# YihongSun/Dynamo-Depth

Measured on AMD Instinct MI355X. Metric: training images/sec (192x640 triplets), higher is better.
Workload: dtype f32

## Files before the change

dynamo-depth_amd/csrc/dd_pw_gemm.hip:

```cpp
#include <hip/hip_runtime.h>
#include <type_traits>

#include "../../include/dynamo_hip.h"
#include "dd_attr.h"
#include "dd_split.h"
#include "dd_store_tile.h"

namespace dd {
namespace pw {

using cm::bf8;
using cm::f16v;
using cm::split2;
using cm::store_acc32;
using cm::StoreF32;
using cm::tile_bias;

constexpr int FRAG_U4 = 64;

struct PackRegion {
  const float* w;
  long long s_n, s_k;
  int N, K, first;
  int fused;
// ... 324 lines not shown
    for (int n = 0; n < NB2; ++n)
      store_acc32<decltype(full)::value>(acc2[n], bv[n], y + (size_t)row * C + n * 32 + (lane & 31), (size_t)C, M - row, StoreF32{});
  };
  if ((int)blockIdx.x * 128 + 128 <= M) tail(std::true_type{});
  else tail(std::false_type{});
}

template <int C>
static int launch_fused(const float* x, const void* pack1, const void* pack2, const float* b1, const float* b2, int M, float* y, hipStream_t stream) {
  constexpr int lds = ((C / 16) * 3 + (C / 32) * 6) * FRAG + 6 * C * 4;
  auto kern = mlp_fwd_kernel<C>;
  static dd::LdsAttrOnce lds_attr;
  if (const int rc = lds_attr.ensure(reinterpret_cast<const void*>(kern), (int)(lds))) return rc;
  hipLaunchKernelGGL(kern, dim3((M + 127) / 128), dim3(256), lds, stream, x, static_cast<const uint4*>(pack1), static_cast<const uint4*>(pack2), b1, b2, M, y);
  return (int)hipGetLastError();
}

constexpr int C3 = 224, KS3 = C3 / 16, NB3 = C3 / 32, NHB3 = 6 * C3 / 32;
constexpr int NF3 = KS3 * 3;
constexpr int BR3 = (NF3 + 3) / 4;
constexpr int MLP3_LDS = 2 * NF3 * FRAG + 6 * C3 * 4;
static_assert(NF3 == NB3 * 6, "both operands of a hidden block have the same number of fragments");

template <int NP>
__global__ __launch_bounds__(256, 1) void mlp_fwd224_kernel(const float* __restrict__ x, const uint4* __restrict__ pack1, const uint4* __restrict__ pack2,
                                                            const float* __restrict__ b1, const float* __restrict__ bias, int M, int S,
                                                            float* __restrict__ dst) {
  extern __shared__ __align__(16) unsigned char smem[];
  unsigned char* const s_w1 = smem;
  unsigned char* const s_w2 = smem + NF3 * FRAG;
  float* const s_b1 = reinterpret_cast<float*>(smem + 2 * NF3 * FRAG);
  const int tid = threadIdx.x, lane = tid & 63, wave = __builtin_amdgcn_readfirstlane(tid >> 6) & 3, hh = lane >> 5;
  const int row0 = (int)blockIdx.x * 128 + wave * 32;
  const int split = (int)blockIdx.y, hb0 = split * NHB3 / S, hb1 = (split + 1) * NHB3 / S;

  for (int i = tid; i < 6 * C3; i += 256) s_b1[i] = b1[i];
  uint4 xf[KS3][3];
  {
    const float* xp = x + (size_t)min(row0 + (lane & 31), M - 1) * C3 + hh * 8;
#pragma unroll
    for (int ks = 0; ks < KS3; ++ks) {
      const float4 v0 = *reinterpret_cast<const float4*>(xp + ks * 16), v1 = *reinterpret_cast<const float4*>(xp + ks * 16 + 4);
      unsigned p[3][4];
      split2(v0.x, v0.y, p[0][0], p[1][0], p[2][0]);
      split2(v0.z, v0.w, p[0][1], p[1][1], p[2][1]);
      split2(v1.x, v1.y, p[0][2], p[1][2], p[2][2]);
      split2(v1.z, v1.w, p[0][3], p[1][3], p[2][3]);
#pragma unroll
      for (int pc = 0; pc < 3; ++pc) xf[ks][pc] = make_uint4(p[pc][0], p[pc][1], p[pc][2], p[pc][3]);
    }
  }
  const unsigned lds0 = (unsigned)reinterpret_cast<size_t>(smem);
  auto dma = [&](const uint4* pack, int hb, unsigned char* s_w) {
    const uint4* src = pack + (size_t)hb * (NF3 * 64) + lane;
#pragma unroll
    for (int r = 0; r < BR3; ++r) {
      const int f = min(wave + 4 * r, NF3 - 1);
      const unsigned dst = __builtin_amdgcn_readfirstlane(lds0 + (unsigned)(s_w - smem) + f * FRAG);
      unsigned keep;
      asm volatile("s_mov_b32 %0, m0\n\ts_mov_b32 m0, %2\n\ts_nop 0\n\tglobal_load_lds_dwordx4 %1, off\n\ts_mov_b32 m0, %0"
                   : "=&s"(keep) : "v"(src + f * 64), "s"(dst) : "memory");
    }
  };
  auto wait_barrier = [&]() { asm volatile("s_waitcnt vmcnt(0) lgkmcnt(0)\n\ts_barrier" ::: "memory"); };

  f16v acc2[NB3];
#pragma unroll
  for (int n = 0; n < NB3; ++n)
#pragma unroll
    for (int r = 0; r < 16; ++r) acc2[n][r] = 0.f;
  auto read_w = [&](const unsigned char* s_w, int f, uint4 (&wf)[3]) {
#pragma unroll
    for (int pc = 0; pc < 3; ++pc) wf[pc] = *reinterpret_cast<const uint4*>(s_w + lane * 16 + (f * 3 + pc) * FRAG);
  };
  float hv[16];
  uint4 hf[2][3];
  auto slice = [&](const f16v& acc, int hb, int i) {
    const int r = i < 11 ? i : i - 3;
    if (i < 11 || (i >= 14 && i < 19)) {
      hv[r] = gelu_erf(acc[r] + s_b1[hb * 32 + 8 * (r >> 2) + 4 * hh + (r & 3)]);
      asm volatile("" : "+v"(hv[r]));
    }
    if (i == 11 || i == 12 || i == 19 || i == 20) {
      const int j = i >= 19, q0 = (i == 12 || i == 20) ? 2 : 0;
      unsigned p[3][2];
#pragma unroll
      for (int q = 0; q < 2; ++q) {
        split2(hv[8 * j + 2 * (q0 + q)], hv[8 * j + 2 * (q0 + q) + 1], p[0][q], p[1][q], p[2][q]);
        asm volatile("" : "+v"(p[0][q]), "+v"(p[1][q]), "+v"(p[2][q]));
      }
#pragma unroll
      for (int pc = 0; pc < 3; ++pc) {
        if (q0 == 0) { hf[j][pc].x = p[pc][0]; hf[j][pc].y = p[pc][1]; }
        else { hf[j][pc].z = p[pc][0]; hf[j][pc].w = p[pc][1]; }
      }
    }
  };
  auto gemm1 = [&](f16v& acc, const f16v& prev, int hb, auto act) {
#pragma unroll
    for (int r = 0; r < 16; ++r) acc[r] = 0.f;
    uint4 wf[2][3];
    read_w(s_w1, 0, wf[0]);
#pragma unroll
    for (int ks = 0; ks < KS3; ++ks) {
      if (ks + 1 < KS3) read_w(s_w1, ks + 1, wf[(ks + 1) & 1]);
#pragma unroll
      for (int t = 6 - NP; t < 6; ++t)
        acc = __builtin_amdgcn_mfma_f32_32x32x16_bf16(__builtin_bit_cast(bf8, wf[ks & 1][cm::kPieceA[t]]), __builtin_bit_cast(bf8, xf[ks][cm::kPieceB[t]]), acc, 0, 0, 0);
      if (decltype(act)::value) slice(prev, hb, ks);
      __builtin_amdgcn_sched_barrier(0);
    }
  };
  auto gemm2 = [&](const f16v& prev, int hb) {
    uint4 wf[2][3];
    read_w(s_w2, 0, wf[0]);
#pragma unroll
    for (int i = 0; i < 2 * NB3; ++i) {
      const int j = i / NB3, n = i - j * NB3;
      if (i + 1 < 2 * NB3) read_w(s_w2, ((i + 1) % NB3) * 2 + (i + 1) / NB3, wf[(i + 1) & 1]);
#pragma unroll
      for (int t = 6 - NP; t < 6; ++t)
        acc2[n] = __builtin_amdgcn_mfma_f32_32x32x16_bf16(__builtin_bit_cast(bf8, hf[j][cm::kPieceA[t]]), __builtin_bit_cast(bf8, wf[i & 1][cm::kPieceB[t]]), acc2[n], 0, 0, 0);
      if (j == 0) slice(prev, hb, 14 + n);
      __builtin_amdgcn_sched_barrier(0);
    }
  };

  float bv[NB3];
#pragma unroll
  for (int n = 0; n < NB3; ++n) bv[n] = tile_bias(bias, n * 32 + (lane & 31), C3, pack2);

  f16v acc1;
  dma(pack1, hb0, s_w1);
  wait_barrier();
  gemm1(acc1, acc1, hb0, std::false_type{});
  wait_barrier();
  dma(pack1, min(hb0 + 1, hb1 - 1), s_w1);
  wait_barrier();
  dma(pack2, hb0, s_w2);
  auto block = [&](int hb, auto more) {
    f16v accn;
    if (decltype(more)::value) gemm1(accn, acc1, hb, std::true_type{});
    else {
#pragma unroll
      for (int i = 0; i < KS3; ++i) slice(acc1, hb, i);
    }
    wait_barrier();
    if (decltype(more)::value) dma(pack1, min(hb + 2, hb1 - 1), s_w1);
    gemm2(acc1, hb);
    if (decltype(more)::value) {
      wait_barrier();
      dma(pack2, hb + 1, s_w2);
#pragma unroll
      for (int r = 0; r < 16; ++r) acc1[r] = accn[r];
    }
  };
  for (int hb = hb0; hb < hb1 - 1; ++hb) block(hb, std::true_type{});
  block(hb1 - 1, std::false_type{});

  float* const out = dst + (size_t)split * M * C3;
  auto tail = [&](auto full) {
    const int row = row0 + 4 * hh;
#pragma unroll
    for (int n = 0; n < NB3; ++n)
      store_acc32<decltype(full)::value>(acc2[n], bv[n], out + (size_t)row * C3 + n * 32 + (lane & 31), (size_t)C3, M - row, StoreF32{});
  };
  if ((int)blockIdx.x * 128 + 128 <= M) tail(std::true_type{});
  else tail(std::false_type{});
}

__global__ __launch_bounds__(256) void mlp_fold224_kernel(const float4* __restrict__ partial, const float4* __restrict__ b2, int S, size_t quads, float4* __restrict__ y) {
  const size_t i = (size_t)blockIdx.x * 256 + threadIdx.x;
  if (i >= quads) return;
  float4 a = b2[i % (C3 / 4)];
  for (int s = 0; s < S; ++s) {
    const float4 p = partial[(size_t)s * quads + i];
    a.x += p.x; a.y += p.y; a.z += p.z; a.w += p.w;
  }
  y[i] = a;
}

static int mlp224_splits(int M) {
  const int groups = (M + 127) / 128, n = 256 / groups;
  return n < 1 ? 1 : n > NHB3 ? NHB3 : n;
}

template <int NP>
static int launch_fused224(const float* x, const void* pack1, const void* pack2, const float* b1, const float* b2, int M, int S, float* y, float* partial,
                           hipStream_t stream) {
  auto kern = mlp_fwd224_kernel<NP>;
  static dd::LdsAttrOnce lds_attr;
  if (const int rc = lds_attr.ensure(reinterpret_cast<const void*>(kern), MLP3_LDS)) return rc;
  hipLaunchKernelGGL(kern, dim3((M + 127) / 128, S), dim3(256), MLP3_LDS, stream, x, static_cast<const uint4*>(pack1), static_cast<const uint4*>(pack2), b1,
                     S == 1 ? b2 : nullptr, M, S, S == 1 ? y : partial);
  if (S == 1) return (int)hipGetLastError();
  const size_t quads = (size_t)M * (C3 / 4);
  hipLaunchKernelGGL(mlp_fold224_kernel, dim3((unsigned)((quads + 255) / 256)), dim3(256), 0, stream, reinterpret_cast<const float4*>(partial),
                     reinterpret_cast<const float4*>(b2), S, quads, reinterpret_cast<float4*>(y));
  return (int)hipGetLastError();
}

__global__ __launch_bounds__(256) void gelu_pair_kernel(const float4* __restrict__ pre, float4* __restrict__ g, float4* __restrict__ post, size_t quads) {
  const size_t i = (size_t)blockIdx.x * 256 + threadIdx.x;
  if (i >= quads) return;
  const float4 x4 = pre[i], g4 = g[i];
  const float xv[4] = {x4.x, x4.y, x4.z, x4.w}, gv[4] = {g4.x, g4.y, g4.z, g4.w};
  float pv[4], dv[4];
#pragma unroll
  for (int e = 0; e < 4; ++e) {
    const float x = xv[e];
    const float er = 1.f + erf_poly(x * 0.70710678118654752440f);
    const float pdf = __expf(-0.5f * x * x) * 0.3989422804014327f;
    pv[e] = (x * 0.5f) * er;
    dv[e] = gv[e] * fmaf(x, pdf, 0.5f * er);
  }
  post[i] = make_float4(pv[0], pv[1], pv[2], pv[3]);
  g[i] = make_float4(dv[0], dv[1], dv[2], dv[3]);
// ... 10 lines not shown
  if (!w1 || !w2 || C < 1 || hidden < 1) return (int)hipErrorInvalidValue;
  PackArgs a;
  a.count = 0;
  a.total = 0;
  bool bad = false;
  auto add = [&](const float* w, long long s_n, long long s_k, int N, int K, void* out, int fused = 0) {
    if (!out) return;
    if (K < 16 || K % 16 || (fused && K % 32)) { bad = true; return; }
    PackRegion& r = a.r[a.count++];
    r.w = w; r.s_n = s_n; r.s_k = s_k; r.N = N; r.K = K; r.first = a.total; r.fused = fused; r.out = static_cast<uint4*>(out);
    a.total += ((N + 31) / 32) * (K / 16);
  };
  add(w1, s1_n, s1_k, hidden, C, pack_fwd1);
  add(w2, s2_n, s2_k, C, hidden, pack_fwd2);
  add(w2, s2_k, s2_n, hidden, C, pack_bwd2);
  add(w1, s1_k, s1_n, C, hidden, pack_bwd1);
  add(w2, s2_n, s2_k, C, hidden, pack_fwd2_fused, 1);
  if (a.count == 0 || bad) return (int)hipErrorInvalidValue;
  for (int i = a.count; i < MAX_REGIONS; ++i) a.r[i] = a.r[0];
  hipLaunchKernelGGL(pw_pack_kernel, dim3((a.total * 64 + 255) / 256), dim3(256), 0, static_cast<hipStream_t>(stream), a);
  return (int)hipGetLastError();
}

extern "C" int dd_mlp_fwd_supported(int C) { return (C == 64 || C == 128 || C == 224) ? 1 : 0; }

extern "C" int dd_mlp_fwd_splits(int M, int C) { return (C == dd::pw::C3 && M >= 1) ? dd::pw::mlp224_splits(M) : 1; }

extern "C" size_t dd_mlp_fwd_workspace_bytes(int M, int C, int splits) {
  if (M < 1 || !dd_mlp_fwd_supported(C) || splits < 0 || splits > dd::pw::NHB3) return 0;
  const int S = splits ? splits : dd_mlp_fwd_splits(M, C);
  return (C == dd::pw::C3 && S > 1) ? (size_t)S * M * C * sizeof(float) : 0;
}

extern "C" int dd_mlp_fwd_n(const float* x, const void* pack_fwd1, const void* pack_fwd2_fused, const float* b1, const float* b2, int M, int C, int products,
                            int splits, float* y, void* workspace, size_t workspace_bytes, void* stream) {
  using namespace dd::pw;
  if (C != C3) return (products == 6 && splits <= 1) ? dd_mlp_fwd(x, pack_fwd1, pack_fwd2_fused, b1, b2, M, C, y, stream) : (int)hipErrorInvalidValue;
  if (!x || !pack_fwd1 || !pack_fwd2_fused || !b1 || !b2 || !y || M < 1 || splits < 0 || splits > NHB3) return (int)hipErrorInvalidValue;
  if (products != 6 && products != 3 && products != 1) return (int)hipErrorInvalidValue;
  if ((reinterpret_cast<unsigned long long>(x) | reinterpret_cast<unsigned long long>(y) | reinterpret_cast<unsigned long long>(b2) |
       reinterpret_cast<unsigned long long>(workspace)) & 15ull)
    return (int)hipErrorInvalidValue;
  const int S = splits ? splits : mlp224_splits(M);
  if (S > 1 && (!workspace || workspace_bytes < dd_mlp_fwd_workspace_bytes(M, C, S))) return (int)hipErrorInvalidValue;
  hipStream_t s = static_cast<hipStream_t>(stream);
  float* part = static_cast<float*>(workspace);
  return products == 6 ? launch_fused224<6>(x, pack_fwd1, pack_fwd2_fused, b1, b2, M, S, y, part, s)
       : products == 3 ? launch_fused224<3>(x, pack_fwd1, pack_fwd2_fused, b1, b2, M, S, y, part, s)
                       : launch_fused224<1>(x, pack_fwd1, pack_fwd2_fused, b1, b2, M, S, y, part, s);
}

extern "C" int dd_mlp_fwd(const float* x, const void* pack_fwd1, const void* pack_fwd2_fused, const float* b1, const float* b2, int M, int C, float* y, void* stream) {
  if (!x || !pack_fwd1 || !pack_fwd2_fused || !b1 || !b2 || !y || M < 1 || (reinterpret_cast<unsigned long long>(x) & 15ull)) return (int)hipErrorInvalidValue;
  hipStream_t s = static_cast<hipStream_t>(stream);
  switch (C) {
    case 64: return dd::pw::launch_fused<64>(x, pack_fwd1, pack_fwd2_fused, b1, b2, M, y, s);
    case 128: return dd::pw::launch_fused<128>(x, pack_fwd1, pack_fwd2_fused, b1, b2, M, y, s);
    case 224: return dd::pw::launch_fused224<6>(x, pack_fwd1, pack_fwd2_fused, b1, b2, M, 1, y, nullptr, s);
    default: return (int)hipErrorInvalidValue;
  }
}

extern "C" int dd_gelu_pair(const float* pre, float* g_inout, float* post, size_t n, void* stream) {
  if (!pre || !g_inout || !post || n == 0 || (n & 3)) return (int)hipErrorInvalidValue;
  if ((reinterpret_cast<unsigned long long>(pre) | reinterpret_cast<unsigned long long>(g_inout) | reinterpret_cast<unsigned long long>(post)) & 15ull)
    return (int)hipErrorInvalidValue;
  const size_t quads = n >> 2;
  hipLaunchKernelGGL(dd::pw::gelu_pair_kernel, dim3((unsigned)((quads + 255) / 256)), dim3(256), 0, static_cast<hipStream_t>(stream),
                     reinterpret_cast<const float4*>(pre), reinterpret_cast<float4*>(g_inout), reinterpret_cast<float4*>(post), quads);
  return (int)hipGetLastError();
}

extern "C" int dd_pw_gemm(const float* x, const void* pack, const float* bias, int M, int K, int N, int gelu_in, float* y, void* stream) {
  using namespace dd::pw;
  if (!x || !pack || !y || M < 1 || K < 32 || K % 32 || N < 1) return (int)hipErrorInvalidValue;
  if ((reinterpret_cast<unsigned long long>(x) & 15ull) || (size_t)M * K >= (1ull << 40) || (size_t)M * N >= (1ull << 40)) return (int)hipErrorInvalidValue;
  hipStream_t s = static_cast<hipStream_t>(stream);
  return gelu_in ? dd::pw::dispatch<true>(x, pack, bias, M, K, N, y, s) : dd::pw::dispatch<false>(x, pack, bias, M, K, N, y, s);
}
```

dynamo-depth_amd/hipops/abi.py:

```python
import ctypes as C

DD_MAX_SCALES = 4
DD_NUM_SRC = 2
DD_ABI_VERSION = 2
DD_MODE_RIGID, DD_MODE_FLOW, DD_MODE_FLOW_MASK = 0, 1, 2
DD_PARTIAL_STRIDE = 40
DD_SUMS_STRIDE = 8

_fp = C.c_void_p


class DDPhotoScale(C.Structure):
    _fields_ = [
        ("shift", C.c_int), ("h", C.c_int), ("w", C.c_int),
        ("w_photo", C.c_float), ("w_cons", C.c_float),
        ("disp", _fp),
        ("flow", _fp * DD_NUM_SRC),
        ("mask", _fp * DD_NUM_SRC),
        ("noise", _fp),
        ("g_disp", _fp),
        ("g_flow", _fp * DD_NUM_SRC),
        ("g_mask", _fp * DD_NUM_SRC),
        ("out_color", _fp * DD_NUM_SRC),
        ("out_sample", _fp * DD_NUM_SRC),
# ... 192 lines not shown
        "dd_conv3x3_mfma_n": (i, [v, v, v, i, i, i, i, i, i, i, v, v]),
        "dd_conv3x3_mfma_flat_supported": (i, [i, i, i, i, i]),
        "dd_conv3x3_mfma_flat_workspace_bytes": (z, [i, i, i, i, i]),
        "dd_conv3x3_mfma_flat": (i, [v, v, v, i, i, i, i, i, v, v, z, v]),
        "dd_conv3x3_mfma_flat_n": (i, [v, v, v, i, i, i, i, i, i, v, v, z, v]),
        "dd_conv3x3_mfma_wgrad_workspace_bytes": (z, [i, i, i, i, i]),
        "dd_conv3x3_mfma_bwd_weight": (i, [v, v, i, i, i, i, i, i, v, v, z, v]),
        "dd_conv3x3_mfma_bwd_weight_n": (i, [v, v, i, i, i, i, i, i, i, v, v, z, v]),
        "dd_conv3x3_half_supported": (i, [i, i]),
        "dd_conv3x3_half_pack_bytes": (z, [i, i]),
        "dd_conv3x3_half_pack": (i, [v, C.c_longlong, C.c_longlong, C.c_longlong, C.c_longlong, i, i, i, v, v, v]),
        "dd_conv3x3_half": (i, [v, v, v, i, i, i, i, i, i, i, v, v]),
        "dd_conv3x3_half_wgrad_workspace_bytes": (z, [i, i, i, i, i]),
        "dd_conv3x3_half_bwd_weight": (i, [v, v, i, i, i, i, i, i, i, v, v, z, v]),
        "dd_pw_gemm_pack_bytes": (z, [i, i]),
        "dd_mlp_pack": (i, [v, C.c_longlong, C.c_longlong, v, C.c_longlong, C.c_longlong, i, i, v, v, v, v, v, v]),
        "dd_mlp_fwd_supported": (i, [i]),
        "dd_mlp_fwd": (i, [v, v, v, v, v, i, i, v, v]),
        "dd_mlp_fwd_splits": (i, [i, i]),
        "dd_mlp_fwd_workspace_bytes": (z, [i, i, i]),
        "dd_mlp_fwd_n": (i, [v, v, v, v, v, i, i, i, i, v, v, z, v]),
        "dd_pw_gemm": (i, [v, v, v, i, i, i, i, v, v]),
        "dd_gelu_pair": (i, [v, v, v, z, v]),
        "dd_linear_wgrad_supported": (i, [i, i, i]),
        "dd_linear_wgrad_workspace_bytes": (z, [i, i, i]),
        "dd_linear_wgrad": (i, [v, v, i, i, i, v, v, v, z, v]),
        "dd_linear_wgrad_n": (i, [v, v, i, i, i, i, v, v, v, z, v]),
        "dd_adam_chunk": (i, []),
        "dd_adam_multi": (i, [v, i, v, i, v, C.c_double, C.c_double, C.c_double, C.c_double, C.c_double, v, v, v]),
        "dd_error_string": (C.c_char_p, [i]),
        "dd_abi_version": (i, []),
    }
    found = []
    for name, (res, args) in sig.items():
        try:
            fn = getattr(lib, name)
        except AttributeError:
            continue
        fn.restype = res
        fn.argtypes = args
        found.append(name)
    return found


EXPORTED = (
    "dd_photo_loss", "dd_photo_workspace_bytes", "dd_photo_timing", "dd_photo_timing_read", "dd_photo_loss_part", "dd_smooth_loss", "dd_smooth_workspace_bytes",
    "dd_ground_loss", "dd_ground_workspace_bytes", "dd_ground_plane", "dd_ground_candidates", "dd_ground_select",
    "dd_assemble_losses", "dd_reg_losses_finish", "dd_fused_loss", "dd_fused_loss_part", "dd_fused_loss_supported", "dd_reg_workspace_bytes", "dd_backproject", "dd_backproject_bwd", "dd_project3d", "dd_project3d_bwd", "dd_project3d_workspace_bytes",
    "dd_ssim", "dd_ssim_bwd", "dd_disp_to_depth", "dd_pose_matrix", "dd_pose_matrix_bwd",
    "dd_channel_sum_nhwc", "dd_channel_sum_workspace_bytes", "dd_reflect_pad1_nhwc", "dd_reflect_pad1_nhwc_bwd",
    "dd_dwconv3x3_nhwc", "dd_dwconv3x3_nhwc_bwd_data", "dd_dwconv3x3_nhwc_bwd_weight", "dd_dwconv3x3_workspace_bytes", "dd_conv3x3_cout1_bwd_data",
    "dd_prepare_frames", "dd_prepare_frames_workspace_bytes", "dd_pyramid_down2", "dd_pack_rgb", "dd_depth_metrics", "dd_depth_metrics_workspace_bytes", "dd_depth_metrics_masked", "dd_depth_metrics_masked_workspace_bytes", "dd_depth_metrics_accumulate", "dd_odom_snippet_count", "dd_odom_snippets", "dd_motion_pr", "dd_fill_contours", "dd_lidar_depth_points", "dd_lidar_depth_points_workspace_bytes", "dd_vis_frame", "dd_vis_flow_tiles", "dd_export_depth", "dd_export_plane_u8", "dd_export_cloud_workspace_bytes", "dd_export_cloud", "dd_bn_act_fwd", "dd_bn_act_bwd", "dd_bn_workspace_bytes",
    "dd_bn_act_fwd_t", "dd_bn_act_bwd_t", "dd_channel_sum_nhwc_t", "dd_reflect_pad1_nhwc_t", "dd_reflect_pad1_nhwc_bwd_t", "dd_up_cat_pad_t", "dd_up_cat_pad_bwd_t",
    "dd_layer_norm_fwd", "dd_layer_norm_bwd", "dd_layer_norm_workspace_bytes", "dd_layer_scale_bwd", "dd_layer_scale_workspace_bytes",
    "dd_jpeg_workspace_bytes", "dd_jpeg_decode", "dd_resize_workspace_bytes", "dd_resize_bicubic", "dd_layer_norm_fwd_t", "dd_layer_norm_bwd_t", "dd_layer_scale_bwd_t", "dd_layer_scale_fwd_t", "dd_dwconv3x3_nhwc_t", "dd_dwconv3x3_nhwc_bwd_data_t",
    "dd_dwconv3x3_nhwc_bwd_weight_t", "dd_adam_chunk", "dd_adam_multi", "dd_conv_small_supported", "dd_conv_small_workspace_bytes",
    "dd_conv_small_fwd", "dd_conv_small_bwd_data", "dd_conv_small_bwd_weight", "dd_conv_head_supported", "dd_conv_head_workspace_bytes", "dd_conv_head_fwd",
    "dd_conv_head_bwd_weight", "dd_redu_supported", "dd_redu_workspace_bytes", "dd_redu_fwd", "dd_redu_bwd_data", "dd_redu_bwd_weight",
    "dd_conv3x3_mfma_supported", "dd_conv3x3_mfma_pack_bytes", "dd_conv3x3_mfma_pack", "dd_conv3x3_mfma_pack_many_job_words",
    "dd_conv3x3_mfma_pack_many_blocks", "dd_conv3x3_mfma_pack_many", "dd_conv3x3_mfma", "dd_conv3x3_mfma_n",
    "dd_conv3x3_mfma_flat_supported", "dd_conv3x3_mfma_flat_workspace_bytes", "dd_conv3x3_mfma_flat", "dd_conv3x3_mfma_flat_n",
    "dd_conv3x3_mfma_wgrad_workspace_bytes", "dd_conv3x3_mfma_bwd_weight", "dd_conv3x3_mfma_bwd_weight_n",
    "dd_conv3x3_half_supported", "dd_conv3x3_half_pack_bytes", "dd_conv3x3_half_pack", "dd_conv3x3_half",
    "dd_conv3x3_half_wgrad_workspace_bytes", "dd_conv3x3_half_bwd_weight",
    "dd_pw_gemm_pack_bytes", "dd_mlp_pack", "dd_pw_gemm", "dd_gelu_pair", "dd_mlp_fwd_supported", "dd_mlp_fwd", "dd_mlp_fwd_splits", "dd_mlp_fwd_workspace_bytes", "dd_mlp_fwd_n",
    "dd_linear_wgrad_supported", "dd_linear_wgrad_workspace_bytes", "dd_linear_wgrad", "dd_linear_wgrad_n",
    "dd_error_string", "dd_abi_version",
)


def fill_photo_args(*, B, H, W, mode, automask, want_grad, min_depth, max_depth, ssim_weight, eps, disp_thr,
                    target, source, K, inv_K, T, ts, g_T, sums, workspace, scales, source_packed=None):
    a = DDPhotoArgs()
    a.abi_version = DD_ABI_VERSION
    a.B, a.H, a.W = B, H, W
    a.num_scales = len(scales)
    a.mode, a.automask, a.want_grad = mode, int(bool(automask)), int(bool(want_grad))
    a.min_depth, a.max_depth, a.ssim_weight, a.eps, a.disp_thr = min_depth, max_depth, ssim_weight, eps, disp_thr
    a.target = ptr(target)
    a.K, a.inv_K = ptr(K), ptr(inv_K)
    a.sums, a.workspace = ptr(sums), ptr(workspace)
    for f in range(DD_NUM_SRC):
        a.source[f] = ptr(source[f])
        a.source_packed[f] = ptr(source_packed[f]) if source_packed is not None else None
        a.T[f] = ptr(T[f])
        a.ts[f] = ptr(ts[f]) if ts is not None else None
        a.g_T[f] = ptr(g_T[f]) if g_T is not None else None
    for s, d in enumerate(scales):
# ... 12 lines not shown
```

dynamo-depth_amd/hipops/functions.py:

```python
import os

import torch

from . import lib as L
from .pack_many import PackSet, _ACTIVE_PACK_SETS, _pack_many_on, pack_many_launches, pack_weights_once_per_forward


def _dev(t, name="tensor"):
    if not t.is_cuda:
        raise L.DynamoHipError("%s must live on the GPU: the Dynamo-Depth loss path has no CPU implementation "
                               "(libdynamo_hip.so is the only backend)" % name)
    if t.dtype != torch.float32:
        raise L.DynamoHipError("%s must be float32, got %s" % (name, t.dtype))
    return t.contiguous()


DTYPE_CODE = {torch.float32: 0, torch.float16: 1, torch.bfloat16: 2}


def _p(t):
    return None if t is None else t.data_ptr()


def _ws(nbytes, device):
# ... 959 lines not shown
        y, w1, b1, w2 = ctx.saved_tensors
        lib = L.load()
        B, H, W, Cc = y.shape
        hid, M = w1.shape[0], B * H * W
        stream = L.current_stream()
        g2 = g.to(torch.float32).contiguous().view(M, Cc)
        y2 = y.view(M, Cc)
        with torch.autocast("cuda", enabled=False):
            pre = torch.addmm(b1, y2, w1.t())
            gpre = torch.mm(g2, w2)
        post = torch.empty_like(pre)
        L.check(lib.dd_gelu_pair(_p(pre), _p(gpre), _p(post), M * hid, stream), "dd_gelu_pair")
        gy = None
        if ctx.needs_input_grad[0]:
            with torch.autocast("cuda", enabled=False):
                gy = torch.mm(gpre, w1).view(B, H, W, Cc)
        return (gy,) + _mlp_param_grads(ctx.needs_input_grad, g2, gpre, y2, post, w1, w2, B, H, W, stream)


def mlp_recompute(y, block):
    return MlpRecomputeFn.apply(y, block.pwconv1.weight, block.pwconv1.bias, block.pwconv2.weight, block.pwconv2.bias)


BN_ACTS = {None: 0, "relu": 1, "gelu": 2}


class BatchNormActFn(torch.autograd.Function):

    @staticmethod
    def forward(ctx, x, weight, bias, running, residual, momentum, eps, act, groups):
        B, Cc, H, W = x.shape
        rows = (B // groups) * H * W
        step = rows * Cc * x.element_size()
        lib = L.load()
        out = torch.empty((B, Cc, H, W), dtype=x.dtype, device=x.device, memory_format=torch.channels_last)
        stats = torch.empty(groups, 2, Cc, dtype=torch.float32, device=x.device)
        nbytes = _ws_bytes("dd_bn_workspace_bytes", Cc)
        ws = _ws(nbytes, x.device)
        code, stream = DTYPE_CODE[x.dtype], L.current_stream()
        xp, op, sp = x.data_ptr(), out.data_ptr(), stats.data_ptr()
        rp = residual.data_ptr() if residual is not None else None
        for g in range(groups):
            rm, rv = running[g] if running is not None else (None, None)
            L.check(lib.dd_bn_act_fwd_t(xp + g * step, rp + g * step if rp is not None else None, rows, Cc, _p(weight), _p(bias), eps, momentum,
                                        _p(rm), _p(rv), sp + g * 8 * Cc, sp + g * 8 * Cc + 4 * Cc, act, op + g * step, code, _p(ws), nbytes, stream),
                    "dd_bn_act_fwd_t")
# ... 158 lines not shown
```

dynamo-depth_amd/networks/depth_encoder.py:

```python
import math
import os

import numpy as np
import torch
import torch.nn as nn
import torch.nn.functional as F

from .layers import BatchNorm2d, Conv2d, conv_cat_aligned, stock_slices


class DropPath(nn.Module):

    def __init__(self, drop_prob=0.0):
        super().__init__()
        self.drop_prob = float(drop_prob)

    def forward(self, x):
        if self.drop_prob == 0.0 or not self.training:
            return x
        return x * self.sample_mask(x)

    def sample_mask(self, x):
        if self.drop_prob == 0.0 or not self.training:
            return None
# ... 146 lines not shown
    def forward_cat(self, parts):
        x = conv_cat_aligned(self.conv, parts)
        return self.bn_gelu(x) if self.bn_act else x


class CDilated(nn.Module):
    def __init__(self, nIn, nOut, kSize, stride=1, d=1, groups=1, bias=False):
        super().__init__()
        self.conv = nn.Conv2d(nIn, nOut, kSize, stride=stride, padding=int((kSize - 1) / 2) * d, bias=bias, dilation=d, groups=groups)

    def forward(self, x):
        c = self.conv
        if (x.is_cuda and c.groups == c.in_channels == c.out_channels and c.kernel_size == (3, 3) and c.stride == (1, 1)
                and c.bias is None and c.padding == c.dilation and c.dilation[0] == c.dilation[1]
                and os.environ.get("DD_STOCK_DWCONV", "0") != "1"):
            from hipops.functions import depthwise_conv3x3
            return depthwise_conv3x3(x, c.weight, c.dilation[0])
        return c(x)


def _mlp_residual(block, y, res):
    B, H, W, Cc = y.shape
    if y.is_cuda and os.environ.get("DD_STOCK_LINEAR_GRAD", "0") != "1":
        from hipops.functions import mlp, mlp_fused, mlp_fused_ok, mlp_ok, mlp_recompute, mlp_recompute_ok, pointwise_linear
        y = y.contiguous()
        if mlp_fused_ok(y, block):
            y = mlp_fused(y, block)
        elif mlp_recompute_ok(y, block):
            y = mlp_recompute(y, block)
        elif mlp_ok(y, block):
            y = mlp(y, block)
        else:
            y = pointwise_linear(block.act(pointwise_linear(y, block.pwconv1)), block.pwconv2)
    else:
        y = block.pwconv2(block.act(block.pwconv1(y.reshape(-1, Cc)))).reshape(B, H, W, Cc)
    drop = block.drop_path.sample_mask(y) if isinstance(block.drop_path, DropPath) else None
    if block.gamma is None:
        return res + (y if drop is None else y * drop)
    if y.is_cuda and os.environ.get("DD_STOCK_LAYER_SCALE", "0") != "1":
        from hipops.functions import layer_scale_residual
        return layer_scale_residual(res, y, block.gamma, drop)
    return torch.addcmul(res, y, block.gamma if drop is None else block.gamma * drop)


class DilatedConv(nn.Module):

    def __init__(self, dim, k, dilation=1, stride=1, drop_path=0.0, layer_scale_init_value=1e-6, expan_ratio=6):
        super().__init__()
        self.ddwconv = CDilated(dim, dim, kSize=k, stride=stride, groups=dim, d=dilation)
        self.bn1 = BatchNorm2d(dim)
# ... 167 lines not shown
```

include/dynamo_hip.h:

```cpp
#ifndef DYNAMO_HIP_H_
#define DYNAMO_HIP_H_

#include <stddef.h>
#include <stdint.h>

#ifdef __cplusplus
extern "C" {
#endif

#define DD_MAX_SCALES 4
#define DD_NUM_SRC 2
#define DD_ABI_VERSION 2

#define DD_MODE_RIGID 0
#define DD_MODE_FLOW 1
#define DD_MODE_FLOW_MASK 2

#define DD_PARTIAL_STRIDE 40
#define DD_SUMS_STRIDE 8

typedef struct DDPhotoScale {
  int shift;
  int h, w;
  float w_photo;
// ... 294 lines not shown

int dd_conv3x3_half_supported(int cin, int cout);
size_t dd_conv3x3_half_pack_bytes(int n_out, int k_in);
int dd_conv3x3_half_pack(const float* weight, long long s_co, long long s_ci, long long s_kh, long long s_kw, int cout, int cin, int dtype,
                         void* pack_fwd, void* pack_bwd_data, void* stream);
int dd_conv3x3_half(const void* x, const void* pack, const float* bias, int B, int Hi, int Wi, int k_in, int n_out, int pad, int dtype, void* y,
                    void* stream);
size_t dd_conv3x3_half_wgrad_workspace_bytes(int B, int Ho, int Wo, int cin, int cout);
int dd_conv3x3_half_bwd_weight(const void* x, const void* g_out, int B, int Hi, int Wi, int cin, int cout, int pad, int dtype, float* g_weight,
                               void* workspace, size_t workspace_bytes, void* stream);

size_t dd_pw_gemm_pack_bytes(int N, int K);
int dd_mlp_pack(const float* w1, long long s1_n, long long s1_k, const float* w2, long long s2_n, long long s2_k, int C, int hidden, void* pack_fwd1,
                void* pack_fwd2, void* pack_bwd2, void* pack_bwd1, void* pack_fwd2_fused, void* stream);
int dd_mlp_fwd_supported(int C);
int dd_mlp_fwd(const float* x, const void* pack_fwd1, const void* pack_fwd2_fused, const float* b1, const float* b2, int M, int C, float* y, void* stream);
int dd_mlp_fwd_splits(int M, int C);
size_t dd_mlp_fwd_workspace_bytes(int M, int C, int splits);
int dd_mlp_fwd_n(const float* x, const void* pack_fwd1, const void* pack_fwd2_fused, const float* b1, const float* b2, int M, int C, int products, int splits,
                 float* y, void* workspace, size_t workspace_bytes, void* stream);
int dd_pw_gemm(const float* x, const void* pack, const float* bias, int M, int K, int N, int gelu_in, float* y, void* stream);
int dd_gelu_pair(const float* pre, float* g_inout, float* post, size_t n, void* stream);

int dd_linear_wgrad_supported(int M, int cout, int cin);
size_t dd_linear_wgrad_workspace_bytes(int M, int cout, int cin);
int dd_linear_wgrad(const float* g_out, const float* x, int M, int cout, int cin, float* g_weight, float* g_bias, void* workspace, size_t workspace_bytes,
                    void* stream);
int dd_linear_wgrad_n(const float* g_out, const float* x, int M, int cout, int cin, int products, float* g_weight, float* g_bias, void* workspace,
                      size_t workspace_bytes, void* stream);

typedef struct DDAdamRecord {
  float* param;
  const float* grad;
  float* exp_avg;
  float* exp_avg_sq;
  float* step;
  long long n;
} DDAdamRecord;
int dd_adam_chunk(void);
int dd_adam_multi(const DDAdamRecord* records, int n_records, const int* block_map, int n_blocks, void* aux, double lr, double beta1, double beta2,
                  double eps, double weight_decay, const float* grad_scale, const float* found_inf, void* stream);

#define DD_VIS_MAX_TILES 16
#define DD_VIS_IMG 0
#define DD_VIS_REF_IMG 1
#define DD_VIS_DISP 2
// ... 31 lines not shown
```

Baseline: 361.3.

## Add fused train-mode MLP forward/backward kernels for C=224 blocks

Adds training and dgrad modes to the fused 224-channel MLP kernel. The training forward stores the GELU output and its derivative alongside the output. The backward fuses the grad-through-fc2, the multiply by the GELU derivative and the grad-through-fc1 in one kernel, streaming the derivative tiles into LDS with async loads. This replaces the recompute or unfused path for large row counts, cutting separate GEMM and elementwise launches and a recompute, at the cost of writing and reading two M×1344 fp32 buffers plus extra LDS.

```diff
diff --git a/dynamo-depth_amd/csrc/dd_pw_gemm.hip b/dynamo-depth_amd/csrc/dd_pw_gemm.hip
--- a/dynamo-depth_amd/csrc/dd_pw_gemm.hip
+++ b/dynamo-depth_amd/csrc/dd_pw_gemm.hip
@@ -1,4 +1,5 @@
 #include <hip/hip_runtime.h>
+#include <initializer_list>
 #include <type_traits>
 
 #include "../../include/dynamo_hip.h"
@@ -370,10 +371,14 @@
 constexpr int MLP3_LDS = 2 * NF3 * FRAG + 6 * C3 * 4;
 static_assert(NF3 == NB3 * 6, "both operands of a hidden block have the same number of fragments");
 
-template <int NP>
+constexpr int MLP_FWD = 0, MLP_TRAIN = 1, MLP_DGRAD = 2;
+constexpr int MLP3_DTILE = 4096;
+
+template <int NP, int MODE>
 __global__ __launch_bounds__(256, 1) void mlp_fwd224_kernel(const float* __restrict__ x, const uint4* __restrict__ pack1, const uint4* __restrict__ pack2,
                                                             const float* __restrict__ b1, const float* __restrict__ bias, int M, int S,
-                                                            float* __restrict__ dst) {
+                                                            float* __restrict__ dst, const float* __restrict__ aux_in, float* __restrict__ out_a,
+                                                            float* __restrict__ out_b) {
   extern __shared__ __align__(16) unsigned char smem[];
   unsigned char* const s_w1 = smem;
   unsigned char* const s_w2 = smem + NF3 * FRAG;
@@ -381,8 +386,12 @@
   const int tid = threadIdx.x, lane = tid & 63, wave = __builtin_amdgcn_readfirstlane(tid >> 6) & 3, hh = lane >> 5;
   const int row0 = (int)blockIdx.x * 128 + wave * 32;
   const int split = (int)blockIdx.y, hb0 = split * NHB3 / S, hb1 = (split + 1) * NHB3 / S;
-
-  for (int i = tid; i < 6 * C3; i += 256) s_b1[i] = b1[i];
+  const bool row_ok = row0 + (lane & 31) < M;
+  const unsigned aoff = (unsigned)min(row0 + (lane & 31), M - 1) * (unsigned)(6 * C3) + 4u * hh;
+  const unsigned char* const s_d = smem + MLP3_LDS + wave * 2 * MLP3_DTILE + lane * 16;
+
+  if (MODE != MLP_DGRAD)
+    for (int i = tid; i < 6 * C3; i += 256) s_b1[i] = b1[i];
   uint4 xf[KS3][3];
   {
     const float* xp = x + (size_t)min(row0 + (lane & 31), M - 1) * C3 + hh * 8;
@@ -399,7 +408,7 @@
     }
   }
   const unsigned lds0 = (unsigned)reinterpret_cast<size_t>(smem);
-  auto dma = [&](const uint4* pack, int hb, unsigned char* s_w) {
+  auto dma = [&](const uint4* pack, int hb, unsigned char* s_w) __attribute__((always_inline)) {
     const uint4* src = pack + (size_t)hb * (NF3 * 64) + lane;
 #pragma unroll
     for (int r = 0; r < BR3; ++r) {
@@ -410,24 +419,61 @@
                    : "=&s"(keep) : "v"(src + f * 64), "s"(dst) : "memory");
     }
   };
-  auto wait_barrier = [&]() { asm volatile("s_waitcnt vmcnt(0) lgkmcnt(0)\n\ts_barrier" ::: "memory"); };
+  auto dma_d = [&](int hb, int buf) __attribute__((always_inline)) {
+    const float* src = aux_in + aoff + hb * 32;
+#pragma unroll
+    for (int q = 0; q < 4; ++q) {
+      const unsigned dst = __builtin_amdgcn_readfirstlane(lds0 + (unsigned)(MLP3_LDS + (wave * 2 + buf) * MLP3_DTILE + q * FRAG));
+      unsigned keep;
+      asm volatile("s_mov_b32 %0, m0\n\ts_mov_b32 m0, %2\n\ts_nop 0\n\tglobal_load_lds_dwordx4 %1, off\n\ts_mov_b32 m0, %0"
+                   : "=&s"(keep) : "v"(src + 8 * q), "s"(dst) : "memory");
+    }
+  };
+  auto wait_barrier = [&]() __attribute__((always_inline)) { asm volatile("s_waitcnt vmcnt(0) lgkmcnt(0)\n\ts_barrier" ::: "memory"); };
 
   f16v acc2[NB3];
 #pragma unroll
   for (int n = 0; n < NB3; ++n)
 #pragma unroll
     for (int r = 0; r < 16; ++r) acc2[n][r] = 0.f;
-  auto read_w = [&](const unsigned char* s_w, int f, uint4 (&wf)[3]) {
+  auto read_w = [&](const unsigned char* s_w, int f, uint4 (&wf)[3]) __attribute__((always_inline)) {
 #pragma unroll
     for (int pc = 0; pc < 3; ++pc) wf[pc] = *reinterpret_cast<const uint4*>(s_w + lane * 16 + (f * 3 + pc) * FRAG);
   };
   float hv[16];
+  float dv[4];
   uint4 hf[2][3];
-  auto slice = [&](const f16v& acc, int hb, int i) {
+  int dbuf = 0;
+  auto store_quad = [&](float* __restrict__ out, int hb, int q, const float* v) __attribute__((always_inline)) {
+    if (row_ok) *reinterpret_cast<float4*>(out + aoff + hb * 32 + 8 * q) = make_float4(v[0], v[1], v[2], v[3]);
+  };
+  auto slice = [&](const f16v& acc, int hb, int i) __attribute__((always_inline)) {
     const int r = i < 11 ? i : i - 3;
     if (i < 11 || (i >= 14 && i < 19)) {
-      hv[r] = gelu_erf(acc[r] + s_b1[hb * 32 + 8 * (r >> 2) + 4 * hh + (r & 3)]);
+      if (MODE == MLP_DGRAD) {
+        if ((r & 3) == 0) {
+          const float4 dq = *reinterpret_cast<const float4*>(s_d + dbuf * MLP3_DTILE + (r >> 2) * FRAG);
+          dv[0] = dq.x; dv[1] = dq.y; dv[2] = dq.z; dv[3] = dq.w;
+        }
+        hv[r] = acc[r] * dv[r & 3];
+      } else {
+        const float v = acc[r] + s_b1[hb * 32 + 8 * (r >> 2) + 4 * hh + (r & 3)];
+        if (MODE == MLP_TRAIN) {
+          const float er = 1.f + erf_poly(v * 0.70710678118654752440f);
+          const float pdf = __expf(-0.5f * v * v) * 0.3989422804014327f;
+          hv[r] = (v * 0.5f) * er;
+          dv[r & 3] = fmaf(v, pdf, 0.5f * er);
+          asm volatile("" : "+v"(dv[r & 3]));
+        } else {
+          hv[r] = gelu_erf(v);
+        }
+      }
       asm volatile("" : "+v"(hv[r]));
+      if (MODE == MLP_TRAIN && (r & 3) == 3) store_quad(out_b, hb, r >> 2, dv);
+    }
+    if (MODE != MLP_FWD && (i == 14 || i == 15 || i == 16 || i == 19)) {
+      const int q = i == 19 ? 3 : i - 14;
+      store_quad(out_a, hb, q, hv + 4 * q);
     }
     if (i == 11 || i == 12 || i == 19 || i == 20) {
       const int j = i >= 19, q0 = (i == 12 || i == 20) ? 2 : 0;
@@ -444,7 +490,7 @@
       }
     }
   };
-  auto gemm1 = [&](f16v& acc, const f16v& prev, int hb, auto act) {
+  auto gemm1 = [&](f16v& acc, const f16v& prev, int hb, auto act) __attribute__((always_inline)) {
 #pragma unroll
     for (int r = 0; r < 16; ++r) acc[r] = 0.f;
     uint4 wf[2][3];
@@ -459,7 +505,7 @@
       __builtin_amdgcn_sched_barrier(0);
     }
   };
-  auto gemm2 = [&](const f16v& prev, int hb) {
+  auto gemm2 = [&](const f16v& prev, int hb) __attribute__((always_inline)) {
     uint4 wf[2][3];
     read_w(s_w2, 0, wf[0]);
 #pragma unroll
@@ -480,14 +526,16 @@
 
   f16v acc1;
   dma(pack1, hb0, s_w1);
+  if (MODE == MLP_DGRAD) dma_d(hb0, 0);
   wait_barrier();
   gemm1(acc1, acc1, hb0, std::false_type{});
   wait_barrier();
   dma(pack1, min(hb0 + 1, hb1 - 1), s_w1);
   wait_barrier();
   dma(pack2, hb0, s_w2);
-  auto block = [&](int hb, auto more) {
+  auto block = [&](int hb, auto more) __attribute__((always_inline)) {
     f16v accn;
+    dbuf = (hb - hb0) & 1;
     if (decltype(more)::value) gemm1(accn, acc1, hb, std::true_type{});
     else {
 #pragma unroll
@@ -495,6 +543,7 @@
     }
     wait_barrier();
     if (decltype(more)::value) dma(pack1, min(hb + 2, hb1 - 1), s_w1);
+    if (MODE == MLP_DGRAD && decltype(more)::value) dma_d(hb + 1, dbuf ^ 1);
     gemm2(acc1, hb);
     if (decltype(more)::value) {
       wait_barrier();
@@ -507,7 +556,7 @@
   block(hb1 - 1, std::false_type{});
 
   float* const out = dst + (size_t)split * M * C3;
-  auto tail = [&](auto full) {
+  auto tail = [&](auto full) __attribute__((always_inline)) {
     const int row = row0 + 4 * hh;
 #pragma unroll
     for (int n = 0; n < NB3; ++n)
@@ -520,7 +569,7 @@
 __global__ __launch_bounds__(256) void mlp_fold224_kernel(const float4* __restrict__ partial, const float4* __restrict__ b2, int S, size_t quads, float4* __restrict__ y) {
   const size_t i = (size_t)blockIdx.x * 256 + threadIdx.x;
   if (i >= quads) return;
-  float4 a = b2[i % (C3 / 4)];
+  float4 a = b2 ? b2[i % (C3 / 4)] : make_float4(0.f, 0.f, 0.f, 0.f);
   for (int s = 0; s < S; ++s) {
     const float4 p = partial[(size_t)s * quads + i];
     a.x += p.x; a.y += p.y; a.z += p.z; a.w += p.w;
@@ -533,14 +582,15 @@
   return n < 1 ? 1 : n > NHB3 ? NHB3 : n;
 }
 
-template <int NP>
+template <int NP, int MODE>
 static int launch_fused224(const float* x, const void* pack1, const void* pack2, const float* b1, const float* b2, int M, int S, float* y, float* partial,
-                           hipStream_t stream) {
-  auto kern = mlp_fwd224_kernel<NP>;
+                           hipStream_t stream, const float* aux_in = nullptr, float* out_a = nullptr, float* out_b = nullptr) {
+  constexpr int lds = MLP3_LDS + (MODE == MLP_DGRAD ? 4 * 2 * MLP3_DTILE : 0);
+  auto kern = mlp_fwd224_kernel<NP, MODE>;
   static dd::LdsAttrOnce lds_attr;
-  if (const int rc = lds_attr.ensure(reinterpret_cast<const void*>(kern), MLP3_LDS)) return rc;
-  hipLaunchKernelGGL(kern, dim3((M + 127) / 128, S), dim3(256), MLP3_LDS, stream, x, static_cast<const uint4*>(pack1), static_cast<const uint4*>(pack2), b1,
-                     S == 1 ? b2 : nullptr, M, S, S == 1 ? y : partial);
+  if (const int rc = lds_attr.ensure(reinterpret_cast<const void*>(kern), lds)) return rc;
+  hipLaunchKernelGGL(kern, dim3((M + 127) / 128, S), dim3(256), lds, stream, x, static_cast<const uint4*>(pack1), static_cast<const uint4*>(pack2), b1,
+                     S == 1 ? b2 : nullptr, M, S, S == 1 ? y : partial, aux_in, out_a, out_b);
   if (S == 1) return (int)hipGetLastError();
   const size_t quads = (size_t)M * (C3 / 4);
   hipLaunchKernelGGL(mlp_fold224_kernel, dim3((unsigned)((quads + 255) / 256)), dim3(256), 0, stream, reinterpret_cast<const float4*>(partial),
@@ -597,6 +647,71 @@
   return (int)hipGetLastError();
 }
 
+extern "C" int dd_mlp_train_pack(const float* w1, long long s1_n, long long s1_k, const float* w2, long long s2_n, long long s2_k, int C, int hidden,
+                                 void* pack_fwd1, void* pack_fwd2_fused, void* pack_bwd2, void* pack_bwd1_fused, void* stream) {
+  using namespace dd::pw;
+  if (!w1 || !w2 || C != C3 || hidden != 6 * C3 || !pack_fwd1 || !pack_fwd2_fused || !pack_bwd2 || !pack_bwd1_fused) return (int)hipErrorInvalidValue;
+  PackArgs a;
+  a.count = 0;
+  a.total = 0;
+  auto add = [&](const float* w, long long s_n, long long s_k, int N, int K, void* out, int fused) {
+    PackRegion& r = a.r[a.count++];
+    r.w = w; r.s_n = s_n; r.s_k = s_k; r.N = N; r.K = K; r.first = a.total; r.fused = fused; r.out = static_cast<uint4*>(out);
+    a.total += ((N + 31) / 32) * (K / 16);
+  };
+  add(w1, s1_n, s1_k, hidden, C, pack_fwd1, 0);
+  add(w2, s2_n, s2_k, C, hidden, pack_fwd2_fused, 1);
+  add(w2, s2_k, s2_n, hidden, C, pack_bwd2, 0);
+  add(w1, s1_k, s1_n, C, hidden, pack_bwd1_fused, 1);
+  for (int i = a.count; i < MAX_REGIONS; ++i) a.r[i] = a.r[0];
+  hipLaunchKernelGGL(pw_pack_kernel, dim3((a.total * 64 + 255) / 256), dim3(256), 0, static_cast<hipStream_t>(stream), a);
+  return (int)hipGetLastError();
+}
+
+extern "C" size_t dd_mlp_train_bwd_workspace_bytes(int M, int C, int splits) {
+  if (M < 1 || C != dd::pw::C3 || splits < 0 || splits > dd::pw::NHB3) return 0;
+  const int S = splits ? splits : dd::pw::mlp224_splits(M);
+  return S > 1 ? (size_t)S * M * C * sizeof(float) : 0;
+}
+
+static bool mlp_train_shape_ok(int M, int C, int products, int splits) {
+  return C == dd::pw::C3 && M >= 1 && M <= (1 << 19) && splits >= 0 && splits <= dd::pw::NHB3 && (products == 6 || products == 3 || products == 1);
+}
+
+static bool aligned16(std::initializer_list<const void*> ps) {
+  unsigned long long bits = 0;
+  for (const void* p : ps) bits |= reinterpret_cast<unsigned long long>(p);
+  return (bits & 15ull) == 0;
+}
+
+extern "C" int dd_mlp_train_fwd(const float* x, const void* pack_fwd1, const void* pack_fwd2_fused, const float* b1, const float* b2, int M, int C,
+                                int products, int splits, float* y, float* h, float* d, void* workspace, size_t workspace_bytes, void* stream) {
+  using namespace dd::pw;
+  if (!x || !pack_fwd1 || !pack_fwd2_fused || !b1 || !b2 || !y || !h || !d || !mlp_train_shape_ok(M, C, products, splits)) return (int)hipErrorInvalidValue;
+  if (!aligned16({x, y, h, d, b2, workspace, pack_fwd1, pack_fwd2_fused})) return (int)hipErrorInvalidValue;
+  const int S = splits ? splits : mlp224_splits(M);
+  if (S > 1 && (!workspace || workspace_bytes < dd_mlp_fwd_workspace_bytes(M, C, S))) return (int)hipErrorInvalidValue;
+  hipStream_t s = static_cast<hipStream_t>(stream);
+  float* part = static_cast<float*>(workspace);
+  return products == 6 ? launch_fused224<6, MLP_TRAIN>(x, pack_fwd1, pack_fwd2_fused, b1, b2, M, S, y, part, s, nullptr, h, d)
+       : products == 3 ? launch_fused224<3, MLP_TRAIN>(x, pack_fwd1, pack_fwd2_fused, b1, b2, M, S, y, part, s, nullptr, h, d)
+                       : launch_fused224<1, MLP_TRAIN>(x, pack_fwd1, pack_fwd2_fused, b1, b2, M, S, y, part, s, nullptr, h, d);
+}
+
+extern "C" int dd_mlp_train_bwd(const float* g, const float* d, const void* pack_bwd2, const void* pack_bwd1_fused, int M, int C, int products, int splits,
+                                float* dx, float* gpre, void* workspace, size_t workspace_bytes, void* stream) {
+  using namespace dd::pw;
+  if (!g || !d || !pack_bwd2 || !pack_bwd1_fused || !dx || !gpre || !mlp_train_shape_ok(M, C, products, splits)) return (int)hipErrorInvalidValue;
+  if (!aligned16({g, d, dx, gpre, workspace, pack_bwd2, pack_bwd1_fused})) return (int)hipErrorInvalidValue;
+  const int S = splits ? splits : mlp224_splits(M);
+  if (S > 1 && (!workspace || workspace_bytes < dd_mlp_train_bwd_workspace_bytes(M, C, S))) return (int)hipErrorInvalidValue;
+  hipStream_t s = static_cast<hipStream_t>(stream);
+  float* part = static_cast<float*>(workspace);
+  return products == 6 ? launch_fused224<6, MLP_DGRAD>(g, pack_bwd2, pack_bwd1_fused, nullptr, nullptr, M, S, dx, part, s, d, gpre, nullptr)
+       : products == 3 ? launch_fused224<3, MLP_DGRAD>(g, pack_bwd2, pack_bwd1_fused, nullptr, nullptr, M, S, dx, part, s, d, gpre, nullptr)
+                       : launch_fused224<1, MLP_DGRAD>(g, pack_bwd2, pack_bwd1_fused, nullptr, nullptr, M, S, dx, part, s, d, gpre, nullptr);
+}
+
 extern "C" int dd_mlp_fwd_supported(int C) { return (C == 64 || C == 128 || C == 224) ? 1 : 0; }
 
 extern "C" int dd_mlp_fwd_splits(int M, int C) { return (C == dd::pw::C3 && M >= 1) ? dd::pw::mlp224_splits(M) : 1; }
@@ -620,9 +735,9 @@
   if (S > 1 && (!workspace || workspace_bytes < dd_mlp_fwd_workspace_bytes(M, C, S))) return (int)hipErrorInvalidValue;
   hipStream_t s = static_cast<hipStream_t>(stream);
   float* part = static_cast<float*>(workspace);
-  return products == 6 ? launch_fused224<6>(x, pack_fwd1, pack_fwd2_fused, b1, b2, M, S, y, part, s)
-       : products == 3 ? launch_fused224<3>(x, pack_fwd1, pack_fwd2_fused, b1, b2, M, S, y, part, s)
-                       : launch_fused224<1>(x, pack_fwd1, pack_fwd2_fused, b1, b2, M, S, y, part, s);
+  return products == 6 ? launch_fused224<6, MLP_FWD>(x, pack_fwd1, pack_fwd2_fused, b1, b2, M, S, y, part, s)
+       : products == 3 ? launch_fused224<3, MLP_FWD>(x, pack_fwd1, pack_fwd2_fused, b1, b2, M, S, y, part, s)
+                       : launch_fused224<1, MLP_FWD>(x, pack_fwd1, pack_fwd2_fused, b1, b2, M, S, y, part, s);
 }
 
 extern "C" int dd_mlp_fwd(const float* x, const void* pack_fwd1, const void* pack_fwd2_fused, const float* b1, const float* b2, int M, int C, float* y, void* stream) {
@@ -631,7 +746,7 @@
   switch (C) {
     case 64: return dd::pw::launch_fused<64>(x, pack_fwd1, pack_fwd2_fused, b1, b2, M, y, s);
     case 128: return dd::pw::launch_fused<128>(x, pack_fwd1, pack_fwd2_fused, b1, b2, M, y, s);
-    case 224: return dd::pw::launch_fused224<6>(x, pack_fwd1, pack_fwd2_fused, b1, b2, M, 1, y, nullptr, s);
+    case 224: return dd::pw::launch_fused224<6, dd::pw::MLP_FWD>(x, pack_fwd1, pack_fwd2_fused, b1, b2, M, 1, y, nullptr, s);
     default: return (int)hipErrorInvalidValue;
   }
 }
diff --git a/dynamo-depth_amd/hipops/abi.py b/dynamo-depth_amd/hipops/abi.py
--- a/dynamo-depth_amd/hipops/abi.py
+++ b/dynamo-depth_amd/hipops/abi.py
@@ -238,6 +238,10 @@
         "dd_mlp_fwd_n": (i, [v, v, v, v, v, i, i, i, i, v, v, z, v]),
         "dd_pw_gemm": (i, [v, v, v, i, i, i, i, v, v]),
         "dd_gelu_pair": (i, [v, v, v, z, v]),
+        "dd_mlp_train_pack": (i, [v, C.c_longlong, C.c_longlong, v, C.c_longlong, C.c_longlong, i, i, v, v, v, v, v]),
+        "dd_mlp_train_fwd": (i, [v, v, v, v, v, i, i, i, i, v, v, v, v, z, v]),
+        "dd_mlp_train_bwd_workspace_bytes": (z, [i, i, i]),
+        "dd_mlp_train_bwd": (i, [v, v, v, v, i, i, i, i, v, v, v, z, v]),
         "dd_linear_wgrad_supported": (i, [i, i, i]),
         "dd_linear_wgrad_workspace_bytes": (z, [i, i, i]),
         "dd_linear_wgrad": (i, [v, v, i, i, i, v, v, v, z, v]),
@@ -280,6 +284,7 @@
     "dd_conv3x3_half_supported", "dd_conv3x3_half_pack_bytes", "dd_conv3x3_half_pack", "dd_conv3x3_half",
     "dd_conv3x3_half_wgrad_workspace_bytes", "dd_conv3x3_half_bwd_weight",
     "dd_pw_gemm_pack_bytes", "dd_mlp_pack", "dd_pw_gemm", "dd_gelu_pair", "dd_mlp_fwd_supported", "dd_mlp_fwd", "dd_mlp_fwd_splits", "dd_mlp_fwd_workspace_bytes", "dd_mlp_fwd_n",
+    "dd_mlp_train_pack", "dd_mlp_train_fwd", "dd_mlp_train_bwd_workspace_bytes", "dd_mlp_train_bwd",
     "dd_linear_wgrad_supported", "dd_linear_wgrad_workspace_bytes", "dd_linear_wgrad", "dd_linear_wgrad_n",
     "dd_error_string", "dd_abi_version",
 )
diff --git a/dynamo-depth_amd/hipops/functions.py b/dynamo-depth_amd/hipops/functions.py
--- a/dynamo-depth_amd/hipops/functions.py
+++ b/dynamo-depth_amd/hipops/functions.py
@@ -1005,6 +1005,76 @@
     return MlpRecomputeFn.apply(y, block.pwconv1.weight, block.pwconv1.bias, block.pwconv2.weight, block.pwconv2.bias)
 
 
+_MLP_TRAIN_CALLS = [0]
+
+_MLP_TRAIN_MIN_ROWS = 1920
+
+
+def mlp_train_calls():
+    return _MLP_TRAIN_CALLS[0]
+
+
+def mlp_train_ok(y, block):
+    if (not torch.is_grad_enabled() or os.environ.get("DD_MLP_TRAIN", "1") != "1" or os.environ.get("DD_STOCK_MLP", "0") == "1"
+            or torch.is_autocast_enabled()):
+        return False
+    l1, l2 = block.pwconv1, block.pwconv2
+    if not (y.is_cuda and y.dtype == torch.float32 and y.dim() == 4 and y.is_contiguous() and y.shape[-1] == 224
+            and l1.weight.dtype == torch.float32 and l2.weight.dtype == torch.float32):
+        return False
+    min_rows = os.environ.get("DD_MLP_TRAIN_MIN_ROWS")
+    if y.shape[0] * y.shape[1] * y.shape[2] < (int(min_rows) if min_rows is not None else _MLP_TRAIN_MIN_ROWS):
+        return False
+    return bool(l1.bias is not None and l2.bias is not None and l1.in_features == 224 and l1.out_features == 6 * 224
+                and l2.in_features == l1.out_features and l2.out_features == 224 and isinstance(block.act, torch.nn.GELU)
+                and getattr(block.act, "approximate", "none") == "none")
+
+
+class MlpTrainFn(torch.autograd.Function):
+
+    @staticmethod
+    def forward(ctx, y, w1, b1, w2, b2):
+        lib = L.load()
+        B, H, W, Cc = y.shape
+        hid, M = w1.shape[0], B * H * W
+        nb = _ws_bytes("dd_pw_gemm_pack_bytes", hid, Cc)
+        packs = torch.empty(nb, dtype=torch.float32, device=y.device)
+        p0, stream = packs.data_ptr(), L.current_stream()
+        L.check(lib.dd_mlp_train_pack(_p(w1), w1.stride(0), w1.stride(1), _p(w2), w2.stride(0), w2.stride(1), Cc, hid, p0, p0 + nb, p0 + 2 * nb,
+                                      p0 + 3 * nb, stream), "dd_mlp_train_pack")
+        out = torch.empty((B, H, W, Cc), dtype=torch.float32, device=y.device)
+        h = torch.empty((M, hid), dtype=torch.float32, device=y.device)
+        d = torch.empty((M, hid), dtype=torch.float32, device=y.device)
+        nbytes = _ws_bytes("dd_mlp_fwd_workspace_bytes", M, Cc, 0)
+        ws = _ws(nbytes, y.device)
+        L.check(lib.dd_mlp_train_fwd(_p(y), p0, p0 + nb, _p(b1), _p(b2), M, Cc, mfma_products(), 0, _p(out), _p(h), _p(d), _p(ws), nbytes, stream),
+                "dd_mlp_train_fwd")
+        _MLP_TRAIN_CALLS[0] += 1
+        ctx.save_for_backward(y, h, d, w1, w2, packs)
+        return out
+
+    @staticmethod
+    def backward(ctx, g):
+        y, h, d, w1, w2, packs = ctx.saved_tensors
+        lib = L.load()
+        B, H, W, Cc = y.shape
+        hid, M = w1.shape[0], B * H * W
+        nb = _ws_bytes("dd_pw_gemm_pack_bytes", hid, Cc)
+        p0, stream = packs.data_ptr(), L.current_stream()
+        g = g.to(torch.float32).contiguous()
+        gy = torch.empty((B, H, W, Cc), dtype=torch.float32, device=g.device)
+        gpre = torch.empty((M, hid), dtype=torch.float32, device=g.device)
+        nbytes = _ws_bytes("dd_mlp_train_bwd_workspace_bytes", M, Cc, 0)
+        ws = _ws(nbytes, g.device)
+        L.check(lib.dd_mlp_train_bwd(_p(g), _p(d), p0 + 2 * nb, p0 + 3 * nb, M, Cc, mfma_products(), 0, _p(gy), _p(gpre), _p(ws), nbytes, stream),
+                "dd_mlp_train_bwd")
+        return (gy if ctx.needs_input_grad[0] else None,) + _mlp_param_grads(ctx.needs_input_grad, g, gpre, y, h, w1, w2, B, H, W, stream)
+
+
+def mlp_train(y, block):
+    return MlpTrainFn.apply(y, block.pwconv1.weight, block.pwconv1.bias, block.pwconv2.weight, block.pwconv2.bias)
+
+
 BN_ACTS = {None: 0, "relu": 1, "gelu": 2}
 
 
diff --git a/dynamo-depth_amd/networks/depth_encoder.py b/dynamo-depth_amd/networks/depth_encoder.py
--- a/dynamo-depth_amd/networks/depth_encoder.py
+++ b/dynamo-depth_amd/networks/depth_encoder.py
@@ -192,10 +192,13 @@
 def _mlp_residual(block, y, res):
     B, H, W, Cc = y.shape
     if y.is_cuda and os.environ.get("DD_STOCK_LINEAR_GRAD", "0") != "1":
-        from hipops.functions import mlp, mlp_fused, mlp_fused_ok, mlp_ok, mlp_recompute, mlp_recompute_ok, pointwise_linear
+        from hipops.functions import (mlp, mlp_fused, mlp_fused_ok, mlp_ok, mlp_recompute, mlp_recompute_ok, mlp_train, mlp_train_ok,
+                                      pointwise_linear)
         y = y.contiguous()
         if mlp_fused_ok(y, block):
             y = mlp_fused(y, block)
+        elif mlp_train_ok(y, block):
+            y = mlp_train(y, block)
         elif mlp_recompute_ok(y, block):
             y = mlp_recompute(y, block)
         elif mlp_ok(y, block):
diff --git a/include/dynamo_hip.h b/include/dynamo_hip.h
--- a/include/dynamo_hip.h
+++ b/include/dynamo_hip.h
@@ -340,6 +340,14 @@
 int dd_pw_gemm(const float* x, const void* pack, const float* bias, int M, int K, int N, int gelu_in, float* y, void* stream);
 int dd_gelu_pair(const float* pre, float* g_inout, float* post, size_t n, void* stream);
 
+int dd_mlp_train_pack(const float* w1, long long s1_n, long long s1_k, const float* w2, long long s2_n, long long s2_k, int C, int hidden, void* pack_fwd1,
+                      void* pack_fwd2_fused, void* pack_bwd2, void* pack_bwd1_fused, void* stream);
+int dd_mlp_train_fwd(const float* x, const void* pack_fwd1, const void* pack_fwd2_fused, const float* b1, const float* b2, int M, int C, int products,
+                     int splits, float* y, float* h, float* d, void* workspace, size_t workspace_bytes, void* stream);
+size_t dd_mlp_train_bwd_workspace_bytes(int M, int C, int splits);
+int dd_mlp_train_bwd(const float* g, const float* d, const void* pack_bwd2, const void* pack_bwd1_fused, int M, int C, int products, int splits, float* dx,
+                     float* gpre, void* workspace, size_t workspace_bytes, void* stream);
+
 int dd_linear_wgrad_supported(int M, int cout, int cin);
 size_t dd_linear_wgrad_workspace_bytes(int M, int cout, int cin);
 int dd_linear_wgrad(const float* g_out, const float* x, int M, int cout, int cin, float* g_weight, float* g_bias, void* workspace, size_t workspace_bytes,
```

Result: faster. 366.5, median of 6 (+1.4%).
